# sm00thix/cvmatrix

Hardware: NVIDIA B200
Metric: fold matrices/sec (higher is better)
Workload: dtype f64

## Files before the change

### cvmatrix_b200/csrc/cvmx_api.cu

```cuda
#include <algorithm>
#include <cstdio>
#include <cstring>
#include <string>
#include <thread>
#include <utility>
#include <vector>

#include "../../include/cvmx.h"
#include "host_stager.h"
#include "kernels_stats.cuh"
#include "kernels_gram.cuh"
#include "kernels_gram_tc.cuh"
#include "kernels_scan.cuh"
#include "kernels_pls.cuh"
#include "kernels_ridge.cuh"
#include <cstdlib>
#include <type_traits>

using namespace cvmx;

namespace {

thread_local std::string g_err;

// ... 61 lines not shown
  TableCache tc_gram, tc_finish;
  DevBuf fold_gram, fold_raw, chunk_ranges;
  int64_t fold_gram_version = -1;
  bool slab = false;
  int64_t N_glob = 0, row0 = 0;
  DevBuf w_glob, g_off, g_idx;
  std::vector<int64_t> g_h_off;
  int slab_scan_mode = 0;
  int slab_scan_stage = 0;
  int64_t slab_scan_f0 = 0, slab_scan_f1 = 0, slab_scan_csr = -1;
  bool mass_started = false;
  bool mass_pending = false;
  bool fit_pre_done = false;
  bool filling = false;
  int64_t fill_units_cap = 0, fill_calls = 0;
  DevBuf ystage;
  DevBuf scan_seg, scan_ok, scan_list, scan_cnt, scan_look, peer_sum;
  int f32_tc = 1;
  int fmap = 0;
  bool attr_tc = false;
  int fuse_stats = 1;
  DevBuf stat_flags;
  HostStager* stager = nullptr;
  int use_stager = 1;
  int scan_spec = 1;
  int64_t scan_launches = 0;
  int64_t launches = 0;
  bool prof = false;
  std::vector<cudaEvent_t> prof_ev;
  std::vector<std::pair<int, std::pair<int, int>>> prof_spans;
  size_t prof_used = 0;
  std::string err;
};

namespace {

int32_t fail(cvmx_t* h, int32_t code, const std::string& msg) {
  if (h) h->err = msg;
  g_err = msg;
  return code;
}

#define CU(h, expr)                                                                                     \
  do {                                                                                                  \
    cudaError_t e__ = (expr);                                                                           \
    if (e__ != cudaSuccess)                                                                             \
      return fail(h, e__ == cudaErrorMemoryAllocation ? CVMX_ERR_NOMEM : CVMX_ERR_CUDA,                  \
                  std::string(#expr) + ": " + cudaGetErrorString(e__));                                 \
  } while (0)

struct DeviceGuard {
  int prev = -1;
  cudaError_t err = cudaSuccess;
  explicit DeviceGuard(int dev) {
    if (cudaGetDevice(&prev) != cudaSuccess) prev = -1;
    if (prev != dev) err = cudaSetDevice(dev); else prev = -1;
  }
  ~DeviceGuard() { if (prev >= 0) cudaSetDevice(prev); }
  DeviceGuard(const DeviceGuard&) = delete;
  DeviceGuard& operator=(const DeviceGuard&) = delete;
};
#define ON_DEVICE(h) DeviceGuard guard__((h)->device); CU(h, guard__.err)

enum { PROF_STATS = 0, PROF_GRAM = 1, PROF_REDUCE = 2, PROF_KINDS = 3 };

int prof_mark(cvmx_t* h) {
  if (!h->prof) return -1;
  if (h->prof_used == h->prof_ev.size()) {
    cudaEvent_t e;
    if (cudaEventCreate(&e) != cudaSuccess) return -1;
    h->prof_ev.push_back(e);
  }
  cudaEventRecord(h->prof_ev[h->prof_used], h->stream);
  return (int)h->prof_used++;
}
void prof_span(cvmx_t* h, int kind, int a, int b) {
  if (h->prof && a >= 0 && b >= 0) h->prof_spans.push_back({kind, {a, b}});
}

inline cudaError_t h2d_copy(cvmx_t* h, void* dst, const void* src, size_t bytes, cudaStream_t stream, bool pageable) {
  if (pageable && h->use_stager && bytes >= ((size_t)4 << 20)) {
    try {
      if (!h->stager) h->stager = new HostStager();
      return h->stager->copy(dst, src, bytes, stream);
    } catch (...) {
      h->use_stager = 0;
    }
  }
  return cudaMemcpyAsync(dst, src, bytes, cudaMemcpyHostToDevice, stream);
}

inline size_t esz(const cvmx_t* h) { return h->dtype == CVMX_F64 ? 8 : 4; }
inline int64_t round_up(int64_t a, int64_t b) { return (a + b - 1) / b * b; }

void plan_tiles(const cvmx_t* h, uint32_t want, std::vector<int2>& tiles) {
  tiles.clear();
  const int64_t TI = (h->K + GB - 1) / GB, TJ = (h->K + h->M + GB - 1) / GB;
  for (int pass = 0; pass < 2; ++pass)
    for (int64_t bi = 0; bi < TI; ++bi)
      for (int64_t bj = bi; bj < TJ; ++bj) {
        const bool first = bi == bj || (bi == 0 && bj >= TI);
        if (first != (pass == 0)) continue;
        const bool has_x = bj * GB < h->K;
        const bool has_y = (bj + 1) * GB > h->K && h->M > 0;
        if (((want & CVMX_WANT_XTX) && has_x) || ((want & CVMX_WANT_XTY) && has_y)) tiles.push_back(make_int2((int)bi, (int)bj));
      }
}

double simulate_makespan(std::vector<int64_t> unit_rows, const std::vector<double>& tile_cost, int64_t sms) {
  std::sort(unit_rows.begin(), unit_rows.end(), std::greater<int64_t>());
  std::vector<double> heap((size_t)sms, 0.0);
  auto cmp = std::greater<double>();
  for (int64_t n : unit_rows)
    for (double c : tile_cost) {
      std::pop_heap(heap.begin(), heap.end(), cmp);
      heap.back() += ((double)n + 1.5 * GBK) * c;
      std::push_heap(heap.begin(), heap.end(), cmp);
    }
  return *std::max_element(heap.begin(), heap.end());
}

std::vector<int64_t> taper_sizes(int64_t n, int64_t R, int levels) {
  std::vector<int64_t> tail;
  int64_t r = R;
  for (int l = 0; l < levels; ++l) { r = std::max<int64_t>(256, (r / 2) / GBK * GBK); tail.push_back(r); tail.push_back(r); }
  int64_t tail_sum = 0;
  for (int64_t t : tail) tail_sum += t;
  std::vector<int64_t> sizes;
  const int64_t main_rows = std::max<int64_t>(0, n - tail_sum);
  if (main_rows > 0) {
    const int64_t k = std::max<int64_t>(1, (main_rows + R / 2) / R), per = round_up((main_rows + k - 1) / k, GBK);
    for (int64_t i = 0; i < k; ++i) {
      const int64_t a = std::min(main_rows, i * per), b = std::min(main_rows, (i + 1) * per);
      if (b > a) sizes.push_back(b - a);
    }
  }
  int64_t rem = n;
  for (int64_t v : sizes) rem -= v;
  for (int64_t t : tail) {
    const int64_t v = std::min(rem, t);
    if (v > 0) { sizes.push_back(v); rem -= v; }
  }
  if (rem > 0) { if (sizes.empty()) sizes.push_back(rem); else sizes.back() += rem; }
  return sizes;
}

std::vector<std::vector<int64_t>> plan_tapered(const std::vector<int64_t>& fold_rows, const std::vector<int2>& tiles, int64_t sms,
                                               int64_t r_lo, int64_t r_hi) {
  struct Memo { std::vector<int64_t> rows; size_t ntiles; int64_t sms; std::vector<std::vector<int64_t>> sizes; };
  static thread_local std::vector<Memo> memo;
  for (const Memo& m : memo)
    if (m.rows == fold_rows && m.ntiles == tiles.size() && m.sms == sms) return m.sizes;
  std::vector<double> tile_cost;
  for (const int2& t : tiles) tile_cost.push_back(t.x == t.y ? 0.78 : 1.0);
  double best = 1e300;
  std::vector<std::vector<int64_t>> best_sizes;
  for (int64_t R = r_lo; R <= r_hi; R += 8 * GBK)
    for (int levels = 2; levels <= 4; ++levels) {
      std::vector<std::vector<int64_t>> sizes;
      std::vector<int64_t> all;
      for (int64_t n : fold_rows) {
        sizes.push_back(n > 0 ? taper_sizes(n, R, levels) : std::vector<int64_t>{0});
        all.insert(all.end(), sizes.back().begin(), sizes.back().end());
      }
      const double mk = simulate_makespan(all, tile_cost, sms);
      if (mk < best - 1e-9) { best = mk; best_sizes = sizes; }
    }
  if (memo.size() >= 8) memo.erase(memo.begin());
  memo.push_back({fold_rows, tiles.size(), sms, best_sizes});
  return best_sizes;
}

void sort_units_longest_first(Plan& pl) {
  std::stable_sort(pl.units.begin(), pl.units.end(),
                   [](const GramUnit& a, const GramUnit& b) { return a.row_end - a.row_begin > b.row_end - b.row_begin; });
  for (size_t i = pl.units.size(); i-- > 0;) pl.fold_units[pl.units[i].fold] = (int32_t)i;
}

void plan_units(const cvmx_t* h, const int64_t* off, int64_t f0, int64_t f1, int ntiles, Plan& pl) {
  const int64_t Pn = f1 - f0;
  pl.units.clear(); pl.fold_units.assign(Pn, 0); pl.split_folds.clear();
  pl.n_partial_units = 0; pl.max_rows = 0;
  const int64_t sms = h->sm_count;
  int64_t rows_per_unit = INT64_MAX;
  if (Pn * ntiles < 8 * sms) {
    double best = -1;
    int64_t total_rows = 0;
    for (int64_t f = f0; f < f1; ++f) total_rows += off[f + 1] - off[f];
    const int64_t max_units = std::max<int64_t>(Pn, (int64_t)(((size_t)2 << 30) / ((size_t)std::max(ntiles, 1) * GACC * GTHREADS * sizeof(double))));
    const int64_t r_min = std::max<int64_t>(2048, round_up((total_rows + max_units - 1) / max_units, GBK));
    for (int64_t R = r_min; R <= r_min + 2048; R += GBK) {
      int64_t items = 0;
      for (int64_t f = f0; f < f1; ++f) items += std::max<int64_t>(1, (off[f + 1] - off[f] + R - 1) / R);
      items *= ntiles;
      const double eff = (double)items / (double)(sms * ((items + sms - 1) / sms));
      if (eff > best + 1e-9) { best = eff; rows_per_unit = R; }
    }
  }
  std::vector<std::vector<int64_t>> tapered;
  if (rows_per_unit != INT64_MAX && ntiles < sms) {
    std::vector<int64_t> fold_rows;
    for (int64_t f = f0; f < f1; ++f) fold_rows.push_back(off[f + 1] - off[f]);
    int64_t r_hi = 8192;
    if (const char* e = std::getenv("CVMX_PLAN_RHI")) r_hi = std::max<int64_t>(1024, std::atoll(e));
    tapered = plan_tapered(fold_rows, pl.tiles, sms, 1024, r_hi);
  }
  for (int64_t f = f0; f < f1; ++f) {
    const int64_t beg = off[f], n = off[f + 1] - off[f];
    pl.max_rows = std::max(pl.max_rows, n);
    std::vector<int64_t> sizes;
    if (!tapered.empty()) sizes = tapered[f - f0];
    else {
      const int64_t ns = (rows_per_unit == INT64_MAX) ? 1 : std::max<int64_t>(1, (n + rows_per_unit - 1) / rows_per_unit);
      const int64_t per = round_up((n + ns - 1) / ns, GBK);
      for (int64_t s = 0; s < ns; ++s) sizes.push_back(std::min(n, (s + 1) * per) - std::min(n, s * per));
    }
    const int64_t ns = (int64_t)sizes.size();
    pl.fold_units[f - f0] = (int32_t)pl.units.size();
    if (ns > 1) pl.split_folds.push_back((int32_t)(f - f0));
    int64_t pos = beg;
    for (int64_t s = 0; s < ns; ++s) {
      GramUnit u;
      u.row_begin = pos; u.row_end = pos + sizes[s];
      pos += sizes[s];
      u.fold = (int32_t)(f - f0); u.split = (int32_t)s; u.nsplit = (int32_t)ns;
      u.part_base = (int32_t)pl.n_partial_units;
      pl.units.push_back(u);
    }
    if (ns > 1) pl.n_partial_units += ns;
  }
  sort_units_longest_first(pl);
}

constexpr double F32_TC_MIN_WIDTH = 65536.0;
template <typename T> int fmap_of(const cvmx_t* h) { return sizeof(T) == 4 ? h->fmap : 0; }
template <typename T> void choose_fmap(cvmx_t* h, int64_t K, int64_t M) {
  h->fmap = (sizeof(T) == 4 && (h->f32_tc == 2 || (h->f32_tc == 1 && (double)K * (double)(K + M) >= F32_TC_MIN_WIDTH))) ? 1 : 0;
}

template <typename T>
int32_t launch_k_gram(cvmx_t* h, unsigned grid, const GramParams<T>& gp) {
  if constexpr (sizeof(T) == 4) {
    if (gp.fmap == 1) {
      if (!h->attr_tc) {
        CU(h, cudaFuncSetAttribute(k_gram_tc, cudaFuncAttributeMaxDynamicSharedMemorySize, (int)gram_tc_smem_bytes()));
        h->attr_tc = true;
      }
      k_gram_tc<<<grid, GLAUNCH, gram_tc_smem_bytes(), h->stream>>>(gp);
      return CVMX_OK;
    }
  }
  if (gp.fuse_stats) {
    if (!h->attr_gram_fused) {
      CU(h, cudaFuncSetAttribute(k_gram<T, true>, cudaFuncAttributeMaxDynamicSharedMemorySize, (int)gram_smem_bytes<T>()));
      h->attr_gram_fused = true;
    }
    k_gram<T, true><<<grid, GLAUNCH, gram_smem_bytes<T>(), h->stream>>>(gp);
    return CVMX_OK;
  }
  k_gram<T><<<grid, GLAUNCH, gram_smem_bytes<T>(), h->stream>>>(gp);
  return CVMX_OK;
}

template <typename T>
int32_t launch_gram(cvmx_t* h, const Plan& pl, const int64_t* d_indices, const EpiParams<T>& epi,
                    cudaEvent_t stats_ready = nullptr, bool fuse_stats = false) {
  const int ntiles = (int)pl.tiles.size();
  if (ntiles == 0 || pl.units.empty()) return CVMX_OK;
  CU(h, h->units.reserve(pl.units.size() * sizeof(GramUnit)));
  CU(h, h->tiles.reserve(pl.tiles.size() * sizeof(int2)));
  CU(h, h->fold_units.reserve(pl.fold_units.size() * sizeof(int32_t)));
  CU(h, cudaMemcpyAsync(h->units.p, pl.units.data(), pl.units.size() * sizeof(GramUnit), cudaMemcpyHostToDevice, h->stream));
  CU(h, cudaMemcpyAsync(h->tiles.p, pl.tiles.data(), pl.tiles.size() * sizeof(int2), cudaMemcpyHostToDevice, h->stream));
  CU(h, cudaMemcpyAsync(h->fold_units.p, pl.fold_units.data(), pl.fold_units.size() * sizeof(int32_t), cudaMemcpyHostToDevice, h->stream));
  if (pl.n_partial_units) {
    CU(h, h->partials.reserve((size_t)pl.n_partial_units * ntiles * GACC * GTHREADS * sizeof(double)));
    CU(h, h->split_folds.reserve(pl.split_folds.size() * sizeof(int32_t)));
    CU(h, cudaMemcpyAsync(h->split_folds.p, pl.split_folds.data(), pl.split_folds.size() * sizeof(int32_t), cudaMemcpyHostToDevice, h->stream));
  }
  GramParams<T> gp;
  gp.fmap = fmap_of<T>(h);
  gp.Z = h->Z.as<T>(); gp.w = h->w.as<T>(); gp.ld = h->ld;
  gp.indices = d_indices;
  gp.units = h->units.as<GramUnit>(); gp.tiles = h->tiles.as<int2>(); gp.ntiles = ntiles;
  gp.partials = h->partials.as<double>();
  gp.raw_out = nullptr; gp.force_partials = 0;
  gp.epi = epi;
  if (fuse_stats) {
    const size_t nf = pl.fold_units.size();
    CU(h, h->stat_flags.reserve(nf * sizeof(int)));
    CU(h, cudaMemsetAsync(h->stat_flags.p, 0, nf * sizeof(int), h->stream));
    const int TI = (int)((h->K + GB - 1) / GB);
    int nchain = 0;
    for (const int2& t : pl.tiles) nchain += t.x == t.y || (t.x == 0 && t.y >= TI);
    gp.fuse_stats = 1; gp.stat_flags = h->stat_flags.as<int>(); gp.stat_target = GPRODUCERS * nchain;
    MomentParams<T>& mp = gp.mom;
    mp.Z = h->Z.as<T>(); mp.w = h->w.as<T>(); mp.ld = h->ld; mp.K = h->K; mp.M = h->M;
    mp.offsets = d_indices; mp.indices = d_indices; mp.fold0 = 0; mp.N = h->N;
    mp.flags = h->flags; mp.resolution = (T)h->resolution;
    mp.sum_z = h->sum_z.as<T>(); mp.sumsq_z = h->sumsq_z.as<T>();
    mp.fs = epi.fs; mp.pw_cols = nullptr; mp.stats = const_cast<T*>(epi.stats); mp.raw = nullptr;
  }
  const size_t smem = gram_smem_bytes<T>();
  if (!h->attr_gram) {
    CU(h, cudaFuncSetAttribute(k_gram<T>, cudaFuncAttributeMaxDynamicSharedMemorySize, (int)smem));
    CU(h, cudaFuncSetAttribute(k_gram_reduce<T>, cudaFuncAttributeMaxDynamicSharedMemorySize, (int)smem));
    h->attr_gram = true;
// ... 2120 lines not shown
```

### cvmatrix_b200/csrc/kernels_gram.cuh

```cuda
#pragma once
#include "common.cuh"
#include "kernels_stats.cuh"

namespace cvmx {

constexpr int GB = 128;
constexpr int GBK = 16;
constexpr int GSTAGES = 4;
constexpr int GTHREADS = 256;
constexpr int GACC = 64;
constexpr int GTILE_ELEMS = GB * GB;

constexpr int GPRODUCERS = 4;
constexpr int GLAUNCH = GTHREADS + 32 * GPRODUCERS;
constexpr int GREGS_PRODUCER = 64;
constexpr int GREGS_COMPUTE = 208;
static_assert(GTHREADS * GREGS_COMPUTE + 32 * GPRODUCERS * GREGS_PRODUCER <= (GTHREADS + 32 * GPRODUCERS) * 168,
              "setmaxnreg budget exceeds the registers the CTA owns");
__device__ __forceinline__ void compute_barrier() { asm volatile("bar.sync 1, %0;\n" ::"n"(GTHREADS) : "memory"); }

template <typename T> struct GramCfg;
template <> struct GramCfg<double> { static constexpr int PITCH = 132; static constexpr int CPITCH = 130; typedef double2 vec2; };
template <> struct GramCfg<float>  { static constexpr int PITCH = 136; static constexpr int CPITCH = 130; typedef float2 vec2; };

// ... 42 lines not shown
__host__ __device__ constexpr size_t gram_smem_bytes() {
  size_t pipe = sizeof(T) * ((size_t)2 * GSTAGES * GBK * GramCfg<T>::PITCH + (size_t)GSTAGES * GBK);
  size_t stage = sizeof(T) * (size_t)GB * GramCfg<T>::CPITCH + 2 * GB * sizeof(double);
  size_t body = (pipe > stage ? pipe : stage);
  return (body + 15) / 16 * 16 + 2 * GSTAGES * sizeof(uint64_t);
}

template <typename T>
__device__ __forceinline__ T gram_scale(T a, double ri, double rj) { return (T)__dmul_rn((double)a, __dmul_rn(ri, rj)); }

template <typename T>
__device__ __forceinline__ void gram_recip_rows(const EpiParams<T>& e, const T* __restrict__ sdev, int64_t i0, int64_t j0, int t, int nthr,
                                                int nrows, double* rrow, double* rcol) {
  const bool sX = e.flags & 4, sY = e.flags & 8;
  const int64_t K = e.K, C = e.K + e.M;
  for (int x = t; x < nrows + GB; x += nthr) {
    const bool row = x < nrows;
    const int64_t col = row ? i0 + x : j0 + (x - nrows);
    const bool on = col < C && (col < K ? sX : sY) && !(row && col >= K);
    const double r = on ? __ddiv_rn(1.0, (double)sdev[col]) : 1.0;
    if (row) rrow[x] = r; else rcol[x - nrows] = r;
  }
}

template <typename T, int U = 16>
__device__ __forceinline__ void gram_epilogue(double (&acc)[8][4][2], T* sC, const EpiParams<T>& e, int fold, int bi,
                                              int bj, int fmap = 0) {
  constexpr int CP = GramCfg<T>::CPITCH;
  typedef typename GramCfg<T>::vec2 vec2;
  const int tid = threadIdx.x, lane = tid & 31, warp = tid >> 5;
  const int wm = warp >> 2, wn = warp & 3, g = lane >> 2, q = lane & 3;
  const int64_t K = e.K, C = e.K + e.M, ld = e.ld;
  const bool diag = bi == bj;

  if (fmap == 1) {
    const int r = 32 * (warp & 3) + lane, cb = 64 * (warp >> 2);
#pragma unroll
    for (int t = 0; t < 8; ++t)
#pragma unroll
      for (int u = 0; u < 4; ++u) {
        vec2 v;
        v.x = (T)acc[t][u][0]; v.y = (T)acc[t][u][1];
        *reinterpret_cast<vec2*>(sC + r * CP + cb + (t * 4 + u) * 2) = v;
      }
  } else {
#pragma unroll
    for (int t = 0; t < 8; ++t) {
      const int r = wm * 64 + 16 * (t >> 1) + 2 * g + (t & 1);
#pragma unroll
      for (int up = 0; up < 2; ++up) {
        const int cb = wn * 32 + up * 16 + 4 * q;
        vec2 lo, hi;
        lo.x = (T)acc[t][2 * up][0]; lo.y = (T)acc[t][2 * up + 1][0];
        hi.x = (T)acc[t][2 * up][1]; hi.y = (T)acc[t][2 * up + 1][1];
        *reinterpret_cast<vec2*>(sC + r * CP + cb) = lo;
        *reinterpret_cast<vec2*>(sC + r * CP + cb + 2) = hi;
      }
    }
  }
  double* rrow = reinterpret_cast<double*>(sC + (size_t)GB * CP);
  double* rcol = rrow + GB;
  if (e.mode == 1 && (e.flags & 12))
    gram_recip_rows<T>(e, e.stats + (size_t)fold * 2 * ld + ld, (int64_t)bi * GB, (int64_t)bj * GB, tid, GTHREADS, GB, rrow, rcol);
  compute_barrier();

  if (e.mode == 1) {
    const bool cX = e.flags & 1, cY = e.flags & 2, sX = e.flags & 4, sY = e.flags & 8;
    const T* __restrict__ mean = e.stats + (size_t)fold * 2 * ld;
    const T* __restrict__ Tt = e.Ttot;
    const T sw = (T)e.fs[fold].sw;
    const int c = (tid & 63) * 2, r0 = tid >> 6;
    const int64_t j = (int64_t)bj * GB + c;
    if (j < C) {
      const vec2 mj = *reinterpret_cast<const vec2*>(mean + j);
      const T mjj[2] = {mj.x, mj.y};
      const double rjj[2] = {rcol[c], rcol[c + 1]};
      const bool isX[2] = {j < K, j + 1 < K};
#pragma unroll 1
      for (int it0 = 0; it0 < GB / 4; it0 += U) {
        vec2 tv[U];
        T mi[U];
        bool ok[U];
#pragma unroll
        for (int u = 0; u < U; ++u) {
          const int r = r0 + 4 * (it0 + u);
          const int64_t i = (int64_t)bi * GB + r;
          ok[u] = i < K && !(diag && c + 1 < r);
          if (ok[u]) {
            tv[u] = __ldg(reinterpret_cast<const vec2*>(Tt + i * ld + j));
            mi[u] = __ldg(mean + i);
          }
        }
#pragma unroll
        for (int u = 0; u < U; ++u) {
          if (!ok[u]) continue;
          const int r = r0 + 4 * (it0 + u);
          vec2 gv = *reinterpret_cast<const vec2*>(sC + r * CP + c);
          T a[2] = {Rn<T>::sub(tv[u].x, gv.x), Rn<T>::sub(tv[u].y, gv.y)};
          const double ri_u = rrow[r];
#pragma unroll
          for (int x = 0; x < 2; ++x) {
            if (isX[x] ? cX : (cX || cY)) a[x] = Rn<T>::sub(a[x], Rn<T>::mul(sw, Rn<T>::mul(mi[u], mjj[x])));
            if (sX || sY) a[x] = gram_scale<T>(a[x], ri_u, rjj[x]);
          }
          gv.x = a[0]; gv.y = a[1];
          *reinterpret_cast<vec2*>(sC + r * CP + c) = gv;
        }
      }
    }
    compute_barrier();
  }

  const bool wxx = e.want & 1, wxy = e.want & 2;
  T* oxx = e.out_xx + (size_t)fold * e.xx_stride;
  T* oxy = e.out_xy + (size_t)fold * e.xy_stride;
  const bool vec_ok = wxx && (e.xx_pitch % 2 == 0) && (e.xx_stride % 2 == 0) &&
                      (reinterpret_cast<uintptr_t>(e.out_xx) % (2 * sizeof(T)) == 0);
#pragma unroll 1
  for (int idx = tid; idx < GTILE_ELEMS / 2; idx += GTHREADS) {
    const int r = idx >> 6, c = (idx & 63) * 2;
    const int64_t i = (int64_t)bi * GB + r, j = (int64_t)bj * GB + c;
    if (i >= K || j >= C) continue;
    vec2 v;
    if (diag && c + 1 < r) { v.x = sC[c * CP + r]; v.y = sC[(c + 1) * CP + r]; }
    else {
      v = *reinterpret_cast<const vec2*>(sC + r * CP + c);
      if (diag && c < r) v.x = sC[c * CP + r];
    }
    if (j + 1 < K && vec_ok) {
      *reinterpret_cast<vec2*>(oxx + i * e.xx_pitch + j) = v;
    } else {
      const T vv[2] = {v.x, v.y};
#pragma unroll
      for (int x = 0; x < 2; ++x) {
        const int64_t jj = j + x;
        if (jj < K) { if (wxx) oxx[i * e.xx_pitch + jj] = vv[x]; }
        else if (jj < C && wxy) oxy[i * e.xy_pitch + (jj - K)] = vv[x];
      }
    }
  }
  if (!diag && wxx) {
#pragma unroll 1
    for (int idx = tid; idx < GTILE_ELEMS / 2; idx += GTHREADS) {
      const int c = (idx >> 7) * 2, r = idx & 127;
      const int64_t i = (int64_t)bi * GB + r, j = (int64_t)bj * GB + c;
      if (i >= K || j >= K) continue;
      const vec2 v = *reinterpret_cast<const vec2*>(sC + r * CP + c);
      oxx[j * e.xx_pitch + i] = v.x;
      if (j + 1 < K) oxx[(j + 1) * e.xx_pitch + i] = v.y;
    }
  }
}

template <typename T, bool FUSE = false>
__global__ void __launch_bounds__(GLAUNCH, 1) k_gram(const GramParams<T> p) {
  extern __shared__ __align__(128) unsigned char smem_raw[];
  constexpr int PITCH = GramCfg<T>::PITCH;
  typedef typename GramCfg<T>::vec2 vec2;

  T* sA = reinterpret_cast<T*>(smem_raw);
  T* sB = sA + (size_t)GSTAGES * GBK * PITCH;
  T* sW = sB + (size_t)GSTAGES * GBK * PITCH;
  uint64_t* full = reinterpret_cast<uint64_t*>(smem_raw + gram_smem_bytes<T>() - 2 * GSTAGES * sizeof(uint64_t));
  uint64_t* empty = full + GSTAGES;

  const int tid = threadIdx.x, lane = tid & 31, warp = tid >> 5;
  const int wm = warp >> 2, wn = warp & 3, g = lane >> 2, q = lane & 3;
  const int tile = blockIdx.x % p.ntiles;
  const GramUnit unit = p.units[blockIdx.x / p.ntiles];
  const int2 tl = p.tiles[tile];
  const int bi = tl.x, bj = tl.y;
  const bool diag = bi == bj;
  const int64_t ld = p.ld;
  const int64_t nrows = unit.row_end - unit.row_begin;
  const int64_t nk = (nrows + GBK - 1) / GBK;

  const bool fused_epi = unit.nsplit == 1 && !p.force_partials;
  const bool chain_tile = FUSE && fused_epi && (diag || (bi == 0 && bj >= (int)((p.epi.K + GB - 1) / GB)));
  if (tid == 0) {
    for (int s = 0; s < GSTAGES; ++s) { mbar_init(full + s, 33); mbar_init(empty + s, GTHREADS / 32 + (chain_tile ? GPRODUCERS : 0)); }
    mbar_fence_init();
  }
  __syncthreads();

  const int pr = lane & 15, po = lane >> 4;
  const int64_t pcol = (int64_t)(po ? bj : bi) * GB;
  const unsigned pbytes = (unsigned)(min((int64_t)GB, ld - pcol) * (int64_t)sizeof(T));
  auto fetch_row = [&](int64_t kt) -> int64_t {
    const int64_t pos = unit.row_begin + kt * GBK + pr;
    if (kt >= nk || pos >= unit.row_end) return -1;
    return p.indices ? p.indices[pos] : pos;
  };
  auto issue = [&](int64_t kt, int64_t grow) {
    if (kt >= nk) return;
    const int slot = (int)(kt % GSTAGES);
    const unsigned round = (unsigned)(kt / GSTAGES);
    if (round > 0) mbar_wait(empty + slot, (round & 1) ^ 1);
    const int rows = (int)min((int64_t)GBK, nrows - kt * GBK);
    if (lane == 0) {
      const unsigned a_bytes = (unsigned)(min((int64_t)GB, ld - (int64_t)bi * GB) * (int64_t)sizeof(T));
      const unsigned b_bytes = diag ? 0u : (unsigned)(min((int64_t)GB, ld - (int64_t)bj * GB) * (int64_t)sizeof(T));
      mbar_arrive_expect_tx(full + slot, (unsigned)rows * (a_bytes + b_bytes));
    }
    if (grow >= 0 && !(diag && po)) {
      T* dst = (po ? sB : sA) + ((size_t)slot * GBK + pr) * PITCH;
      bulk_g2s(dst, p.Z + grow * ld + pcol, pbytes, full + slot);
    }
    if (po == 0) {
      if (sizeof(T) == 8) cp_async8(sW + slot * GBK + pr, p.w + (grow >= 0 ? grow : 0), grow >= 0 ? 8 : 0);
      else cp_async4(sW + slot * GBK + pr, p.w + (grow >= 0 ? grow : 0), grow >= 0 ? 4 : 0);
    }
    cp_async_mbar_arrive_noinc(full + slot);
  };

  if (warp >= GTHREADS / 32) {
    asm volatile("setmaxnreg.dec.sync.aligned.u32 %0;\n" ::"n"(GREGS_PRODUCER));
    const int pw = warp - GTHREADS / 32;
    if (FUSE && chain_tile) {
      static_assert(GSTAGES == GPRODUCERS, "one producer warp per ring slot");
      int64_t mine = pw;
      int64_t row = fetch_row(mine);
      if (mine < nk) { const int64_t nr = fetch_row(mine + GPRODUCERS); issue(mine, row); row = nr; mine += GPRODUCERS; }
      T cs = T(0), cq = T(0);
      const int col = pw * 32 + lane;
#pragma unroll 1
      for (int64_t j = 0; j < nk; ++j) {
        const int slot = (int)(j % GSTAGES);
        mbar_wait(full + slot, (unsigned)(j / GSTAGES) & 1);
        const T* zc = (diag ? sA : sB) + (size_t)slot * GBK * PITCH + col;
        const T* wb = sW + slot * GBK;
        const int rows = (int)min((int64_t)GBK, nrows - j * GBK);
#pragma unroll 4
        for (int k = 0; k < rows; ++k) {
          const T z = zc[k * PITCH];
          const T t = Rn<T>::mul(z, wb[k]);
          cs = Rn<T>::add(cs, t);
          cq = Rn<T>::add(cq, Rn<T>::mul(t, z));
        }
        __syncwarp();
        if (lane == 0) mbar_arrive(empty + slot);
        if (mine == j + GSTAGES - 1 && mine < nk) { const int64_t nr = fetch_row(mine + GPRODUCERS); issue(mine, row); row = nr; mine += GPRODUCERS; }
      }
      finalize_column<T>(p.mom, unit.fold, (int64_t)bj * GB + col, cs, cq);
      __threadfence();
      __syncwarp();
      if (lane == 0) atomicAdd(p.stat_flags + unit.fold, 1);
      cp_async_wait<0>();
      return;
    }
    int64_t kt = pw;
    int64_t row = fetch_row(kt);
#pragma unroll 1
    for (; kt < nk; kt += GPRODUCERS) {
      const int64_t next_row = fetch_row(kt + GPRODUCERS);
      issue(kt, row);
      row = next_row;
    }
    cp_async_wait<0>();
    return;
  }
  asm volatile("setmaxnreg.inc.sync.aligned.u32 %0;\n" ::"n"(GREGS_COMPUTE));

  double acc[8][4][2];
#pragma unroll
  for (int t = 0; t < 8; ++t)
#pragma unroll
    for (int u = 0; u < 4; ++u) acc[t][u][0] = acc[t][u][1] = 0.0;

  const bool half = diag && wm == 1;
  const bool helper = half && wn < 2;
  const int ewn = helper ? wn + 2 : wn;
  const int my_parity = helper ? 1 : 0;

#pragma unroll 1
  for (int64_t kt = 0; kt < nk; ++kt) {
    const int slot = (int)(kt % GSTAGES);
    mbar_wait(full + slot, (unsigned)(kt / GSTAGES) & 1);
    const T* a_base = sA + (size_t)slot * GBK * PITCH + wm * 64 + 2 * g;
    const T* b_base = (diag ? sA : sB) + (size_t)slot * GBK * PITCH + ewn * 32 + 2 * g;
    const T* w_base = sW + slot * GBK;
    const int rows = (int)min((int64_t)GBK, nrows - kt * GBK);
    if (half && (int)(kt & 1) != my_parity) {
    } else if (rows == GBK) {
#pragma unroll
      for (int kk = 0; kk < GBK / 4; ++kk) {
        const int k = kk * 4 + q;
        const T wv = w_base[k];
        double a[8], b[4];
#pragma unroll
        for (int tp = 0; tp < 4; ++tp) {
          const vec2 v = *reinterpret_cast<const vec2*>(a_base + k * PITCH + tp * 16);
          a[2 * tp] = (double)Rn<T>::mul(v.x, wv);
          a[2 * tp + 1] = (double)Rn<T>::mul(v.y, wv);
        }
#pragma unroll
        for (int up = 0; up < 2; ++up) {
          const vec2 v = *reinterpret_cast<const vec2*>(b_base + k * PITCH + up * 16);
          b[2 * up] = (double)v.x;
          b[2 * up + 1] = (double)v.y;
        }
#pragma unroll
        for (int t = 0; t < 8; ++t)
#pragma unroll
          for (int u = 0; u < 4; ++u) dmma884(acc[t][u][0], acc[t][u][1], a[t], b[u]);
      }
    } else {
#pragma unroll 1
      for (int kk = 0; kk * 4 < rows; ++kk) {
        const int k = kk * 4 + q;
        const bool ok = k < rows;
        const T wv = ok ? w_base[k] : T(0);
        double a[8], b[4];
#pragma unroll
        for (int tp = 0; tp < 4; ++tp) {
          vec2 v; v.x = T(0); v.y = T(0);
          if (ok) v = *reinterpret_cast<const vec2*>(a_base + k * PITCH + tp * 16);
          a[2 * tp] = ok ? (double)Rn<T>::mul(v.x, wv) : 0.0;
          a[2 * tp + 1] = ok ? (double)Rn<T>::mul(v.y, wv) : 0.0;
        }
#pragma unroll
        for (int up = 0; up < 2; ++up) {
          vec2 v; v.x = T(0); v.y = T(0);
          if (ok) v = *reinterpret_cast<const vec2*>(b_base + k * PITCH + up * 16);
          b[2 * up] = (double)v.x;
          b[2 * up + 1] = (double)v.y;
        }
#pragma unroll
        for (int t = 0; t < 8; ++t)
#pragma unroll
          for (int u = 0; u < 4; ++u) dmma884(acc[t][u][0], acc[t][u][1], a[t], b[u]);
      }
    }
    __syncwarp();
    if (lane == 0) mbar_arrive(empty + slot);
  }
  if (FUSE && fused_epi) {
    if (tid == 0) {
      int seen;
      do {
        asm volatile("ld.acquire.gpu.global.s32 %0, [%1];\n" : "=r"(seen) : "l"(p.stat_flags + unit.fold) : "memory");
        if (seen < p.stat_target) __nanosleep(64);
      } while (seen < p.stat_target);
    }
  }
  compute_barrier();

  if (diag) {
    double* hbuf = reinterpret_cast<double*>(smem_raw);
    if (helper) {
      double* dst = hbuf + (size_t)wn * GACC * 32 + lane;
#pragma unroll
      for (int t = 0; t < 8; ++t)
#pragma unroll
        for (int u = 0; u < 4; ++u) {
          dst[((t * 4 + u) * 2 + 0) * 32] = acc[t][u][0];
          dst[((t * 4 + u) * 2 + 1) * 32] = acc[t][u][1];
          acc[t][u][0] = acc[t][u][1] = 0.0;
        }
    }
    compute_barrier();
    if (half && !helper) {
      const double* src = hbuf + (size_t)(wn - 2) * GACC * 32 + lane;
#pragma unroll
      for (int t = 0; t < 8; ++t)
#pragma unroll
        for (int u = 0; u < 4; ++u) {
          acc[t][u][0] += src[((t * 4 + u) * 2 + 0) * 32];
          acc[t][u][1] += src[((t * 4 + u) * 2 + 1) * 32];
        }
    }
    compute_barrier();
  }

  if (fused_epi) {
    gram_epilogue<T>(acc, reinterpret_cast<T*>(smem_raw), p.epi, unit.fold, bi, bj);
  } else {
    double* dst = p.partials + ((size_t)(unit.part_base + unit.split) * p.ntiles + tile) * (size_t)(GACC * GTHREADS);
#pragma unroll
    for (int t = 0; t < 8; ++t)
#pragma unroll
      for (int u = 0; u < 4; ++u) {
        dst[((t * 4 + u) * 2 + 0) * GTHREADS + tid] = acc[t][u][0];
        dst[((t * 4 + u) * 2 + 1) * GTHREADS + tid] = acc[t][u][1];
      }
  }
}

template <typename T>
__global__ void __launch_bounds__(GTHREADS, 1) k_gram_reduce(const GramParams<T> p, const int32_t* __restrict__ fold_units,
                                                             const int32_t* __restrict__ fold_list) {
  extern __shared__ __align__(128) unsigned char smem_raw[];
  const int tid = threadIdx.x;
  const int tile = blockIdx.x;
  const int fold = fold_list[blockIdx.y];
  const GramUnit unit = p.units[fold_units[fold]];
  const int2 tl = p.tiles[tile];
  double acc[8][4][2];
  const size_t tile_off = ((size_t)unit.part_base * p.ntiles + tile) * (size_t)(GACC * GTHREADS);
  const double* src = (p.npeers > 0 ? p.peers[0] : p.partials) + tile_off;
  const size_t split_stride = (size_t)p.ntiles * GACC * GTHREADS;
#pragma unroll
  for (int t = 0; t < 8; ++t)
#pragma unroll
    for (int u = 0; u < 4; ++u) {
      acc[t][u][0] = src[((t * 4 + u) * 2 + 0) * GTHREADS + tid];
      acc[t][u][1] = src[((t * 4 + u) * 2 + 1) * GTHREADS + tid];
    }
  if (p.npeers > 0) {
#pragma unroll
    for (int t = 0; t < 8; ++t)
#pragma unroll
      for (int u = 0; u < 4; ++u) {
        double v0[7], v1[7];
#pragma unroll
        for (int q = 1; q < 8; ++q) {
          const bool on = q < p.npeers;
          v0[q - 1] = on ? (p.peers[q] + tile_off)[((t * 4 + u) * 2 + 0) * GTHREADS + tid] : 0.0;
          v1[q - 1] = on ? (p.peers[q] + tile_off)[((t * 4 + u) * 2 + 1) * GTHREADS + tid] : 0.0;
        }
#pragma unroll
        for (int q = 1; q < 8; ++q) { acc[t][u][0] += v0[q - 1]; acc[t][u][1] += v1[q - 1]; }
      }
  } else {
    for (int s = 1; s < unit.nsplit; ++s) {
      const double* ps = src + s * split_stride;
#pragma unroll
      for (int t = 0; t < 8; ++t)
#pragma unroll
        for (int u = 0; u < 4; ++u) {
          acc[t][u][0] += ps[((t * 4 + u) * 2 + 0) * GTHREADS + tid];
          acc[t][u][1] += ps[((t * 4 + u) * 2 + 1) * GTHREADS + tid];
        }
    }
  }
  if (p.raw_out) {
    double* dst = p.raw_out + ((size_t)unit.fold * p.ntiles + tile) * (size_t)(GACC * GTHREADS);
#pragma unroll
    for (int t = 0; t < 8; ++t)
#pragma unroll
      for (int u = 0; u < 4; ++u) {
        dst[((t * 4 + u) * 2 + 0) * GTHREADS + tid] = acc[t][u][0];
        dst[((t * 4 + u) * 2 + 1) * GTHREADS + tid] = acc[t][u][1];
      }
    return;
  }
  gram_epilogue<T>(acc, reinterpret_cast<T*>(smem_raw), p.epi, unit.fold, tl.x, tl.y, p.fmap);
}

__global__ void __launch_bounds__(256) k_partial_sum(const double* __restrict__ partials, const GramUnit* __restrict__ units,
                                                     const int32_t* __restrict__ fold_units, int ntiles, double* __restrict__ out) {
  const int fold = blockIdx.z, tile = blockIdx.y;
  const GramUnit unit = units[fold_units[fold]];
  const size_t tile_elems = (size_t)GACC * GTHREADS, split_stride = (size_t)ntiles * tile_elems;
  const size_t e = ((size_t)blockIdx.x * 256 + threadIdx.x) * 2;
  const double* src = partials + ((size_t)unit.part_base * ntiles + tile) * tile_elems + e;
  double2 acc = *reinterpret_cast<const double2*>(src);
  int s = 1;
  for (; s + 4 <= unit.nsplit; s += 4) {
    double2 v[4];
#pragma unroll
    for (int u = 0; u < 4; ++u) v[u] = *reinterpret_cast<const double2*>(src + (size_t)(s + u) * split_stride);
#pragma unroll
    for (int u = 0; u < 4; ++u) { acc.x += v[u].x; acc.y += v[u].y; }
  }
  for (; s < unit.nsplit; ++s) {
    const double2 v = *reinterpret_cast<const double2*>(src + (size_t)s * split_stride);
    acc.x += v.x; acc.y += v.y;
  }
  *reinterpret_cast<double2*>(out + ((size_t)unit.fold * ntiles + tile) * tile_elems + e) = acc;
}

struct PeerList { const double* p[8]; };
template <typename T>
__global__ void k_peer_sum_rows(const PeerList peers, int npeers, int64_t offset, int64_t n, T* __restrict__ out) {
  const int64_t i = (int64_t)blockIdx.x * blockDim.x + threadIdx.x;
  if (i >= n) return;
  double v[8];
#pragma unroll
  for (int q = 0; q < 8; ++q) v[q] = q < npeers ? peers.p[q][offset + i] : 0.0;
  double r = 0.0;
#pragma unroll
  for (int q = 0; q < 8; ++q) r += v[q];
  out[i] = (T)r;
}

__global__ void __launch_bounds__(256) k_peer_sum_frags(const PeerList peers, int npeers, int64_t offset, int64_t n, double* __restrict__ out) {
  const int64_t e = ((int64_t)blockIdx.x * blockDim.x + threadIdx.x) * 2;
  if (e >= n) return;
  double2 v[8];
#pragma unroll
  for (int q = 0; q < 8; ++q) v[q] = q < npeers ? *reinterpret_cast<const double2*>(peers.p[q] + offset + e) : make_double2(0.0, 0.0);
  double2 r = v[0];
#pragma unroll
  for (int q = 1; q < 8; ++q) { r.x += v[q].x; r.y += v[q].y; }
  *reinterpret_cast<double2*>(out + e) = r;
}

__global__ void k_normalize_indices(int64_t* __restrict__ idx, int64_t n, int64_t N, int32_t* __restrict__ err) {
  const int64_t i = (int64_t)blockIdx.x * blockDim.x + threadIdx.x;
  if (i >= n) return;
  int64_t v = idx[i];
  if (v < 0) v += N;
  if (v < 0 || v >= N) { *err = 1; v = 0; }
  idx[i] = v;
}

template <typename T>
__global__ void k_repack(const T* __restrict__ src, int64_t rows, int64_t cols, T* __restrict__ dst, int64_t ld) {
  const int64_t total = rows * cols;
  for (int64_t e = (int64_t)blockIdx.x * blockDim.x + threadIdx.x; e < total; e += (int64_t)gridDim.x * blockDim.x) {
    const int64_t r = e / cols, c = e - r * cols;
    dst[r * ld + c] = src[e];
  }
}

template <typename T>
__global__ void k_zero_pad(T* __restrict__ Z, int64_t rows, int64_t ld, int64_t c0) {
  const int64_t w = ld - c0;
  const int64_t total = rows * w;
  for (int64_t e = (int64_t)blockIdx.x * blockDim.x + threadIdx.x; e < total; e += (int64_t)gridDim.x * blockDim.x) {
    const int64_t r = e / w, c = e - r * w;
    Z[r * ld + c0 + c] = T(0);
  }
// ... 466 lines not shown
```

Baseline: 526.0.

## Redistribute diagonal Gram tile work by 16x16 bands across warps

For diagonal Gram tiles, each compute warp now handles a compile-time mask of 16x16 output bands instead of the old scheme where two helper warps split K-tiles by parity. Only bands on or above the diagonal are computed, spread evenly at nine per SM sub-partition. Two warps compute bands owned by other warps, and those results are handed over through shared memory. The aim is to skip the redundant lower-triangle DMMA work and balance tensor-core load, at the cost of more template instantiations and code size. The diagonal tile cost weight in the planner is nudged to match.

```diff
diff --git a/cvmatrix_b200/csrc/cvmx_api.cu b/cvmatrix_b200/csrc/cvmx_api.cu
--- a/cvmatrix_b200/csrc/cvmx_api.cu
+++ b/cvmatrix_b200/csrc/cvmx_api.cu
@@ -237,7 +237,7 @@
   for (const Memo& m : memo)
     if (m.rows == fold_rows && m.ntiles == tiles.size() && m.sms == sms) return m.sizes;
   std::vector<double> tile_cost;
-  for (const int2& t : tiles) tile_cost.push_back(t.x == t.y ? 0.78 : 1.0);
+  for (const int2& t : tiles) tile_cost.push_back(t.x == t.y ? 0.79 : 1.0);
   double best = 1e300;
   std::vector<std::vector<int64_t>> best_sizes;
   for (int64_t R = r_lo; R <= r_hi; R += 8 * GBK)
diff --git a/cvmatrix_b200/csrc/kernels_gram.cuh b/cvmatrix_b200/csrc/kernels_gram.cuh
--- a/cvmatrix_b200/csrc/kernels_gram.cuh
+++ b/cvmatrix_b200/csrc/kernels_gram.cuh
@@ -218,11 +218,133 @@
   }
 }
 
+constexpr int GBANDS_ALL = 0xFF;
+constexpr int GDIAG_MASK[8] = {0x0B, 0xBF, 0xFC, 0xC0, 0x3F, 0x03, 0x0B, 0xBF};
+constexpr int GDIAG_OWNER4 = 3, GDIAG_OWNER5 = 2;
+constexpr bool gdiag_bands_ok() {
+  int cover[8][8] = {}, smsp[4] = {};
+  for (int w = 0; w < 8; ++w) {
+    const int tile = w == 4 ? GDIAG_OWNER4 : w == 5 ? GDIAG_OWNER5 : w;
+    for (int band = 0; band < 8; ++band)
+      if ((GDIAG_MASK[w] >> band) & 1) {
+        ++cover[(tile >> 2) * 4 + band / 2][(tile & 3) * 2 + band % 2];
+        ++smsp[w % 4];
+      }
+  }
+  for (int r = 0; r < 8; ++r)
+    for (int c = 0; c < 8; ++c)
+      if (cover[r][c] != (r <= c ? 1 : 0)) return false;
+  for (int s = 0; s < 4; ++s)
+    if (smsp[s] != 9) return false;
+  return GDIAG_MASK[6] == GDIAG_MASK[0] && GDIAG_MASK[7] == GDIAG_MASK[1];
+}
+static_assert(gdiag_bands_ok(), "diagonal-tile bands: each band on or above the diagonal exactly once, 9 per sub-partition");
+
+template <int MASK> __device__ __forceinline__ constexpr bool gram_band(int t, int u) { return (MASK >> ((t >> 1) * 2 + (u >> 1))) & 1; }
+
+template <typename T, int MASK>
+__device__ __forceinline__ void gram_rows(double (&acc)[8][4][2], const T* sA, const T* sB, const T* sW, uint64_t* full,
+                                          uint64_t* empty, int64_t nrows, int r0, int c0) {
+  constexpr int PITCH = GramCfg<T>::PITCH;
+  typedef typename GramCfg<T>::vec2 vec2;
+  const int lane = threadIdx.x & 31, g = lane >> 2, q = lane & 3;
+#pragma unroll 1
+  for (int64_t kt = 0; kt * GBK < nrows; ++kt) {
+    const int slot = (int)(kt % GSTAGES);
+    mbar_wait(full + slot, (unsigned)(kt / GSTAGES) & 1);
+    const T* a_base = sA + (size_t)slot * GBK * PITCH + r0 + 2 * g;
+    const T* b_base = sB + (size_t)slot * GBK * PITCH + c0 + 2 * g;
+    const T* w_base = sW + slot * GBK;
+    const int rows = (int)min((int64_t)GBK, nrows - kt * GBK);
+    if (rows == GBK) {
+#pragma unroll
+      for (int kk = 0; kk < GBK / 4; ++kk) {
+        const int k = kk * 4 + q;
+        const T wv = w_base[k];
+        double a[8], b[4];
+#pragma unroll
+        for (int tp = 0; tp < 4; ++tp) {
+          if (!((MASK >> (2 * tp)) & 3)) continue;
+          const vec2 v = *reinterpret_cast<const vec2*>(a_base + k * PITCH + tp * 16);
+          a[2 * tp] = (double)Rn<T>::mul(v.x, wv);
+          a[2 * tp + 1] = (double)Rn<T>::mul(v.y, wv);
+        }
+#pragma unroll
+        for (int up = 0; up < 2; ++up) {
+          if (!(MASK & (0x55 << up))) continue;
+          const vec2 v = *reinterpret_cast<const vec2*>(b_base + k * PITCH + up * 16);
+          b[2 * up] = (double)v.x;
+          b[2 * up + 1] = (double)v.y;
+        }
+#pragma unroll
+        for (int t = 0; t < 8; ++t)
+#pragma unroll
+          for (int u = 0; u < 4; ++u)
+            if (gram_band<MASK>(t, u)) dmma884(acc[t][u][0], acc[t][u][1], a[t], b[u]);
+      }
+    } else {
+#pragma unroll 1
+      for (int kk = 0; kk * 4 < rows; ++kk) {
+        const int k = kk * 4 + q;
+        const bool ok = k < rows;
+        const T wv = ok ? w_base[k] : T(0);
+        double a[8], b[4];
+#pragma unroll
+        for (int tp = 0; tp < 4; ++tp) {
+          if (!((MASK >> (2 * tp)) & 3)) continue;
+          vec2 v; v.x = T(0); v.y = T(0);
+          if (ok) v = *reinterpret_cast<const vec2*>(a_base + k * PITCH + tp * 16);
+          a[2 * tp] = ok ? (double)Rn<T>::mul(v.x, wv) : 0.0;
+          a[2 * tp + 1] = ok ? (double)Rn<T>::mul(v.y, wv) : 0.0;
+        }
+#pragma unroll
+        for (int up = 0; up < 2; ++up) {
+          if (!(MASK & (0x55 << up))) continue;
+          vec2 v; v.x = T(0); v.y = T(0);
+          if (ok) v = *reinterpret_cast<const vec2*>(b_base + k * PITCH + up * 16);
+          b[2 * up] = (double)v.x;
+          b[2 * up + 1] = (double)v.y;
+        }
+#pragma unroll
+        for (int t = 0; t < 8; ++t)
+#pragma unroll
+          for (int u = 0; u < 4; ++u)
+            if (gram_band<MASK>(t, u)) dmma884(acc[t][u][0], acc[t][u][1], a[t], b[u]);
+      }
+    }
+    __syncwarp();
+    if (lane == 0) mbar_arrive(empty + slot);
+  }
+}
+
+template <int MASK>
+__device__ __forceinline__ void gram_bands_out(double (&acc)[8][4][2], double* buf) {
+#pragma unroll
+  for (int t = 0; t < 8; ++t)
+#pragma unroll
+    for (int u = 0; u < 4; ++u)
+      if (gram_band<MASK>(t, u)) {
+        buf[((t * 4 + u) * 2 + 0) * 32] = acc[t][u][0];
+        buf[((t * 4 + u) * 2 + 1) * 32] = acc[t][u][1];
+        acc[t][u][0] = acc[t][u][1] = 0.0;
+      }
+}
+template <int MASK>
+__device__ __forceinline__ void gram_bands_in(double (&acc)[8][4][2], const double* buf) {
+#pragma unroll
+  for (int t = 0; t < 8; ++t)
+#pragma unroll
+    for (int u = 0; u < 4; ++u)
+      if (gram_band<MASK>(t, u)) {
+        acc[t][u][0] = buf[((t * 4 + u) * 2 + 0) * 32];
+        acc[t][u][1] = buf[((t * 4 + u) * 2 + 1) * 32];
+      }
+}
+
 template <typename T, bool FUSE = false>
 __global__ void __launch_bounds__(GLAUNCH, 1) k_gram(const GramParams<T> p) {
   extern __shared__ __align__(128) unsigned char smem_raw[];
   constexpr int PITCH = GramCfg<T>::PITCH;
-  typedef typename GramCfg<T>::vec2 vec2;
 
   T* sA = reinterpret_cast<T*>(smem_raw);
   T* sB = sA + (size_t)GSTAGES * GBK * PITCH;
@@ -231,7 +353,7 @@
   uint64_t* empty = full + GSTAGES;
 
   const int tid = threadIdx.x, lane = tid & 31, warp = tid >> 5;
-  const int wm = warp >> 2, wn = warp & 3, g = lane >> 2, q = lane & 3;
+  const int wm = warp >> 2, wn = warp & 3;
   const int tile = blockIdx.x % p.ntiles;
   const GramUnit unit = p.units[blockIdx.x / p.ntiles];
   const int2 tl = p.tiles[tile];
@@ -333,72 +455,19 @@
 #pragma unroll
     for (int u = 0; u < 4; ++u) acc[t][u][0] = acc[t][u][1] = 0.0;
 
-  const bool half = diag && wm == 1;
-  const bool helper = half && wn < 2;
-  const int ewn = helper ? wn + 2 : wn;
-  const int my_parity = helper ? 1 : 0;
-
-#pragma unroll 1
-  for (int64_t kt = 0; kt < nk; ++kt) {
-    const int slot = (int)(kt % GSTAGES);
-    mbar_wait(full + slot, (unsigned)(kt / GSTAGES) & 1);
-    const T* a_base = sA + (size_t)slot * GBK * PITCH + wm * 64 + 2 * g;
-    const T* b_base = (diag ? sA : sB) + (size_t)slot * GBK * PITCH + ewn * 32 + 2 * g;
-    const T* w_base = sW + slot * GBK;
-    const int rows = (int)min((int64_t)GBK, nrows - kt * GBK);
-    if (half && (int)(kt & 1) != my_parity) {
-    } else if (rows == GBK) {
-#pragma unroll
-      for (int kk = 0; kk < GBK / 4; ++kk) {
-        const int k = kk * 4 + q;
-        const T wv = w_base[k];
-        double a[8], b[4];
-#pragma unroll
-        for (int tp = 0; tp < 4; ++tp) {
-          const vec2 v = *reinterpret_cast<const vec2*>(a_base + k * PITCH + tp * 16);
-          a[2 * tp] = (double)Rn<T>::mul(v.x, wv);
-          a[2 * tp + 1] = (double)Rn<T>::mul(v.y, wv);
-        }
-#pragma unroll
-        for (int up = 0; up < 2; ++up) {
-          const vec2 v = *reinterpret_cast<const vec2*>(b_base + k * PITCH + up * 16);
-          b[2 * up] = (double)v.x;
-          b[2 * up + 1] = (double)v.y;
-        }
-#pragma unroll
-        for (int t = 0; t < 8; ++t)
-#pragma unroll
-          for (int u = 0; u < 4; ++u) dmma884(acc[t][u][0], acc[t][u][1], a[t], b[u]);
-      }
-    } else {
-#pragma unroll 1
-      for (int kk = 0; kk * 4 < rows; ++kk) {
-        const int k = kk * 4 + q;
-        const bool ok = k < rows;
-        const T wv = ok ? w_base[k] : T(0);
-        double a[8], b[4];
-#pragma unroll
-        for (int tp = 0; tp < 4; ++tp) {
-          vec2 v; v.x = T(0); v.y = T(0);
-          if (ok) v = *reinterpret_cast<const vec2*>(a_base + k * PITCH + tp * 16);
-          a[2 * tp] = ok ? (double)Rn<T>::mul(v.x, wv) : 0.0;
-          a[2 * tp + 1] = ok ? (double)Rn<T>::mul(v.y, wv) : 0.0;
-        }
-#pragma unroll
-        for (int up = 0; up < 2; ++up) {
-          vec2 v; v.x = T(0); v.y = T(0);
-          if (ok) v = *reinterpret_cast<const vec2*>(b_base + k * PITCH + up * 16);
-          b[2 * up] = (double)v.x;
-          b[2 * up + 1] = (double)v.y;
-        }
-#pragma unroll
-        for (int t = 0; t < 8; ++t)
-#pragma unroll
-          for (int u = 0; u < 4; ++u) dmma884(acc[t][u][0], acc[t][u][1], a[t], b[u]);
-      }
-    }
-    __syncwarp();
-    if (lane == 0) mbar_arrive(empty + slot);
+  if (!diag) {
+    gram_rows<T, GBANDS_ALL>(acc, sA, sB, sW, full, empty, nrows, wm * 64, wn * 32);
+  } else {
+    const int src = warp == 4 ? GDIAG_OWNER4 : warp == 5 ? GDIAG_OWNER5 : warp;
+    const int r0 = (src >> 2) * 64, c0 = (src & 3) * 32;
+    switch (warp) {
+      case 0: case 6: gram_rows<T, GDIAG_MASK[0]>(acc, sA, sA, sW, full, empty, nrows, r0, c0); break;
+      case 1: case 7: gram_rows<T, GDIAG_MASK[1]>(acc, sA, sA, sW, full, empty, nrows, r0, c0); break;
+      case 2: gram_rows<T, GDIAG_MASK[2]>(acc, sA, sA, sW, full, empty, nrows, r0, c0); break;
+      case 3: gram_rows<T, GDIAG_MASK[3]>(acc, sA, sA, sW, full, empty, nrows, r0, c0); break;
+      case 4: gram_rows<T, GDIAG_MASK[4]>(acc, sA, sA, sW, full, empty, nrows, r0, c0); break;
+      default: gram_rows<T, GDIAG_MASK[5]>(acc, sA, sA, sW, full, empty, nrows, r0, c0); break;
+    }
   }
   if (FUSE && fused_epi) {
     if (tid == 0) {
@@ -413,28 +482,11 @@
 
   if (diag) {
     double* hbuf = reinterpret_cast<double*>(smem_raw);
-    if (helper) {
-      double* dst = hbuf + (size_t)wn * GACC * 32 + lane;
-#pragma unroll
-      for (int t = 0; t < 8; ++t)
-#pragma unroll
-        for (int u = 0; u < 4; ++u) {
-          dst[((t * 4 + u) * 2 + 0) * 32] = acc[t][u][0];
-          dst[((t * 4 + u) * 2 + 1) * 32] = acc[t][u][1];
-          acc[t][u][0] = acc[t][u][1] = 0.0;
-        }
-    }
+    if (warp == 4) gram_bands_out<GDIAG_MASK[4]>(acc, hbuf + lane);
+    if (warp == 5) gram_bands_out<GDIAG_MASK[5]>(acc, hbuf + (size_t)GACC * 32 + lane);
     compute_barrier();
-    if (half && !helper) {
-      const double* src = hbuf + (size_t)(wn - 2) * GACC * 32 + lane;
-#pragma unroll
-      for (int t = 0; t < 8; ++t)
-#pragma unroll
-        for (int u = 0; u < 4; ++u) {
-          acc[t][u][0] += src[((t * 4 + u) * 2 + 0) * 32];
-          acc[t][u][1] += src[((t * 4 + u) * 2 + 1) * 32];
-        }
-    }
+    if (warp == GDIAG_OWNER4) gram_bands_in<GDIAG_MASK[4]>(acc, hbuf + lane);
+    if (warp == GDIAG_OWNER5) gram_bands_in<GDIAG_MASK[5]>(acc, hbuf + (size_t)GACC * 32 + lane);
     compute_barrier();
   }
 
```

Result: faster. 571.3 (median of 6 runs) (+8.6%).
